# DefTruth/CUDA-Learn-Notes

Hardware: AMD Instinct MI355X
Metric: HGEMM fp16 TFLOPS at M=N=K=4096 (higher is better)
Workload: dtype f16; 1 GPU; HGEMM fp16 NN M=N=K=4096, stages=2, block swizzle stride 2048 (BASELINE config C3); kernel=hgemm_mma_m16n8k16_mma2x4_warp4x4x2_stages_dsmem, parallelism=replicas x1, launch=eager

## Files before the change

### cuda-learn-notes_amd/csrc/hgemm_w4.cuh

```cuda
#pragma once
#include <type_traits>

#include "hgemm_mfma.cuh"

namespace hgemm {

template <int FM, int FN, int NT = 0>
__device__ __forceinline__ void store_wide_tile_via_lds(half_t* Cmat, int N, int row0, int col0, int lane, char* wave_lds,
                                                        const f4 (&acc)[FM][FN], int nt_ok = 1) {
  static_assert(FN == 8 || FN == 6 || FN == 5 || FN == 4, "128-, 96-, 80- or 64-column wave tile");
  constexpr int RS = FN * 32 + 16;
  constexpr int LPR = FN * 2;
  constexpr int RPI = 64 / LPR;
#pragma unroll
  for (int h0 = 0; h0 < FM; h0 += 4) {
    constexpr int NF_FULL = 4;
    const int nf = FM - h0 < NF_FULL ? FM - h0 : NF_FULL;
#pragma unroll
    for (int i = 0; i < NF_FULL; ++i)
#pragma unroll
      for (int j = 0; j < FN; ++j) {
        if (i < nf) {
          const f4 v = acc[(h0 + i) < FM ? (h0 + i) : 0][j];
          h4 o = {(half_t)v[0], (half_t)v[1], (half_t)v[2], (half_t)v[3]};
          *reinterpret_cast<h4*>(wave_lds + (i * 16 + (lane & 15)) * RS + (j * 16 + 4 * (lane >> 4)) * 2) = o;
        }
      }
    const int rows = nf * 16;
#pragma unroll
    for (int it = 0; it < (64 + RPI - 1) / RPI; ++it) {
      const int r = it * RPI + lane / LPR;
      if (it * RPI < rows && lane < RPI * LPR && r < rows) {
        const u4 v = *reinterpret_cast<const u4*>(wave_lds + r * RS + (lane % LPR) * 16);
        u4* dst = reinterpret_cast<u4*>(Cmat + (size_t)(row0 + h0 * 16 + r) * N + col0 + (lane % LPR) * 8);
        if constexpr (NT == 1) {
          if (nt_ok) asm volatile("global_store_dwordx4 %0, %1, off nt\n\ts_nop 1" ::"v"(dst), "v"(v) : "memory");
          else asm volatile("global_store_dwordx4 %0, %1, off\n\ts_nop 1" ::"v"(dst), "v"(v) : "memory");
        } else if constexpr (NT == 3) asm volatile("global_store_dwordx4 %0, %1, off nt\n\ts_nop 1" ::"v"(dst), "v"(v) : "memory");
        else if constexpr (NT == 2) asm volatile("global_store_dwordx4 %0, %1, off sc0 sc1\n\ts_nop 1" ::"v"(dst), "v"(v) : "memory");
        else *dst = v;
      }
    }
  }
}

template <int FM, int FN>
__device__ __forceinline__ void store_wide_tile_via_lds_rows16(half_t* Cmat, int N, int row0, int col0, int lane, char* wave_lds, const f4 (&acc)[FM][FN],
                                                               int nt_ok) {
  static_assert(FN == 8, "128-column wave tile");
  constexpr int RS = FN * 32 + 16, LPR = FN * 2, RPI = 64 / LPR;
#pragma unroll
  for (int i = 0; i < FM; ++i) {
#pragma unroll
    for (int j = 0; j < FN; ++j) {
      const f4 v = acc[i][j];
      h4 o = {(half_t)v[0], (half_t)v[1], (half_t)v[2], (half_t)v[3]};
      *reinterpret_cast<h4*>(wave_lds + (lane & 15) * RS + (j * 16 + 4 * (lane >> 4)) * 2) = o;
    }
#pragma unroll
    for (int it = 0; it < 16 / RPI; ++it) {
      const int r = it * RPI + lane / LPR;
      const u4 v = *reinterpret_cast<const u4*>(wave_lds + r * RS + (lane % LPR) * 16);
      u4* dst = reinterpret_cast<u4*>(Cmat + (size_t)(row0 + i * 16 + r) * N + col0 + (lane % LPR) * 8);
      if (nt_ok) asm volatile("global_store_dwordx4 %0, %1, off nt\n\ts_nop 1" ::"v"(dst), "v"(v) : "memory");
      else asm volatile("global_store_dwordx4 %0, %1, off\n\ts_nop 1" ::"v"(dst), "v"(v) : "memory");
    }
    asm volatile("s_waitcnt lgkmcnt(0)" ::: "memory");
  }
}

template <int... Ns, typename F>
__device__ __forceinline__ void static_for_impl(std::integer_sequence<int, Ns...>, F&& f) {
  (f(std::integral_constant<int, Ns>{}), ...);
}
template <int N, typename F>
__device__ __forceinline__ void static_for(F&& f) {
  static_for_impl(std::make_integer_sequence<int, N>{}, f);
}

struct W4Sched {
  int r1_first, r1_step;
  int b1;
  int d_first, d_step;
  int b2;
  int r0_first, r0_step;
};
constexpr W4Sched w4_sched(int var) {
  switch (var) {
    case 1: return {1, 2, 36, 38, 4, 94, 96, 2};
    case 2: return {1, 2, 40, 42, 3, 94, 96, 2};
    case 3: return {1, 1, 24, 26, 4, 94, 96, 2};
    case 4: return {1, 2, 36, 38, 4, 102, 103, 1};
    case 5: return {1, 2, 36, 38, 5, 102, 103, 1};
    case 6: return {1, 1, 20, 22, 6, 102, 103, 1};
    case 7: return {1, 2, 36, 38, 4, 94, 95, 1};
    case 8: return {1, 1, 20, 22, 4, 94, 95, 1};
    case 9: return {1, 1, 20, 22, 5, 102, 103, 1};
    case 10: return {1, 2, 36, 38, 8, 102, 103, 1};
    case 11: return {1, 2, 36, 38, 7, 102, 103, 1};
    case 12: return {1, 2, 36, 40, 6, 102, 103, 1};
    case 13: return {1, 1, 36, 38, 4, 102, 103, 1};
    case 14: return {1, 1, 20, 38, 4, 102, 103, 1};
    default: return {1, 2, 40, 42, 2, 94, 96, 2};
  }
}
constexpr W4Sched w4_sched_for(int FM, int FN, int d_step) {
  const int NR = FM + FN, NM = 2 * FM * FN, b1 = 1 + 2 * (NR - 1) + 5, b2 = NM - NR - 10;
  return {1, 2, b1, b1 + 2, d_step, b2, b2 + 1, 1};
}

template <typename C, int NLOADS>
struct NFillW {
  unsigned voff[NLOADS];
  __device__ __forceinline__ void init(int N, int wave, int lane) {
    constexpr int LPR = C::BN / 8;
#pragma unroll
    for (int i = 0; i < NLOADS; ++i) {
      const int L = (i * C::NW + wave) * 64 + lane;
      const int krow = L / LPR, c = L % LPR;
      voff[i] = ((unsigned)krow * (unsigned)N + ((c ^ nswz_bn<C::BN>(krow)) << 3)) * 2u;
    }
  }
};
template <int BN>
__device__ __forceinline__ h8 read_nfrag_w(const char* img, int n0w, int lane, int kk) {
  const int i = lane & 15, g = lane >> 4;
  const int q = (n0w >> 3) + ((i & 3) >> 1);
  const int k_lo = kk * 32 + 8 * g + (i >> 2);
  const int k_hi = k_lo + 4;
  const char* p_lo = img + k_lo * (BN * 2) + ((q ^ nswz_bn<BN>(k_lo)) << 4) + ((i & 1) << 3);
  const char* p_hi = img + k_hi * (BN * 2) + ((q ^ nswz_bn<BN>(k_hi)) << 4) + ((i & 1) << 3);
  return h8_cat(lds_read_tr16(p_lo), lds_read_tr16(p_hi));
}

template <int BM_, int BN_, int LAYOUT_>
struct W4Cfg {
  static constexpr int BM = BM_, BN = BN_, BK = 64, NW = 4, LAYOUT = LAYOUT_;
  static constexpr int WTM = BM / 2, WTN = BN / 2, FM = WTM / 16, FN = WTN / 16;
  static constexpr int A_BYTES = BM * 128, B_BYTES = BN * 128, STAGE_BYTES = A_BYTES + B_BYTES, LDS_BYTES = 2 * STAGE_BYTES;
  static constexpr int A_LOADS = FM, B_LOADS = FN, NP = FM + FN;
  static constexpr int NR = FM + FN, NM = 2 * FM * FN;
  static_assert(((BM == 256 || BM == 192 || BM == 128) && (BN == 256 || BN == 192 || BN == 128) && BM + BN >= 384) ||
                    (BM == 160 && BN == 160),
                "wave tiles of 128, 96, 80 or 64 rows / columns; enough MFMAs per K tile to hang the schedule on");
};

constexpr int W4_TICKET_FLOATS = 1024;
template <int LAYOUT, int EPI = 2, int VAR = 0, int ABL = 0, int BM = 256, int BN = 256, bool ODD = false>
__global__ __launch_bounds__(256, 1) void hgemm_w4_kernel(const half_t* __restrict__ A, const half_t* __restrict__ B,
                                                          half_t* __restrict__ Cmat, int M, int N, int K, int tiles_m,
                                                          int tiles_n, int swizzle, int band, float* __restrict__ ws = nullptr) {
  using C = W4Cfg<BM, BN, LAYOUT>;
  constexpr bool SPLITK = EPI == 5 || EPI == 6;
  constexpr int FM = C::FM, FN = C::FN, NR = C::NR, NP = C::NP, NM = C::NM;
  constexpr W4Sched S = (BM == 256 && BN == 256) ? w4_sched(VAR & 15) : w4_sched_for(FM, FN, (BM == 128 || BN == 128 || BM == 160) ? 2 : (BM == 192 && BN == 192) ? 4 : 5);
  constexpr bool SNAKE = (VAR >> 4) & 1;
  static_assert(S.r0_first + (NR - 1) * S.r0_step < NM && S.r1_first + (NR - 1) * S.r1_step < S.b1 && S.b1 < S.d_first &&
                    S.b2 < S.r0_first && S.r0_first >= NM / 2 && (NP - 1) * S.d_step < NM && S.d_first + (NP - 1) * S.d_step - NM < S.d_first &&
                    S.d_first < NM && S.b2 >= S.d_first,
                "schedule: reads drained before B1, DMA after B1 and landed before the next B2, late pieces before early ones");
  constexpr int D_EARLY = (NM - 1 - S.d_first) / S.d_step + 1 > NP ? NP : (NM - 1 - S.d_first) / S.d_step + 1;
  constexpr int D_BEFORE_B2 = (S.b2 - S.d_first) / S.d_step + 1 > D_EARLY ? D_EARLY : (S.b2 - S.d_first) / S.d_step + 1;
  extern __shared__ __attribute__((aligned(16))) char smem[];
  const int lane = threadIdx.x & 63;
  const int wave = __builtin_amdgcn_readfirstlane(threadIdx.x >> 6);
  const int wm = wave >> 1, wn = wave & 1;
  constexpr bool PERSIST = EPI == 7;
  const int n_tiles = tiles_m * tiles_n;
  int tm, tn;
  auto coords = [&](int vb, int& tm_, int& tn_) {
    if (swizzle & 4) {
      tile_coords_interleaved(vb, PERSIST ? n_tiles : (int)gridDim.x, tiles_m, tiles_n, band, tm_, tn_);
    } else {
      tile_coords(vb, PERSIST ? n_tiles : (int)gridDim.x, tiles_m, tiles_n, swizzle & 1, band, tm_, tn_);
    }
  };
  int vb = blockIdx.x;
  coords(vb, tm, tn);
  int m0 = tm * BM, n0 = tn * BN;

  KFill<C, FM> fa;
  KFill<C, FN> fbt;
  NFillW<C, FN> fbn;
  const char* a_src;
  const char* b_src;
  if constexpr (SPLITK) {
    const int ld = (swizzle >> 8) * 64;
    const size_t k0 = (size_t)blockIdx.y * K;
    fa.init(ld, wave, lane);
    if constexpr (LAYOUT == TN) fbt.init(ld, wave, lane);
    else fbn.init(N, wave, lane);
    a_src = reinterpret_cast<const char*>(A + (size_t)m0 * ld + k0);
    b_src = (LAYOUT == TN) ? reinterpret_cast<const char*>(B + (size_t)n0 * ld + k0) : reinterpret_cast<const char*>(B + k0 * N + n0);
  } else {
    fa.init(K, wave, lane);
    if constexpr (LAYOUT == TN) fbt.init(K, wave, lane);
    else fbn.init(N, wave, lane);
    a_src = reinterpret_cast<const char*>(A + (size_t)m0 * K);
    b_src = (LAYOUT == TN) ? reinterpret_cast<const char*>(B + (size_t)n0 * K) : reinterpret_cast<const char*>(B + n0);
  }
  const size_t a_step = 128;
  const size_t b_step = (LAYOUT == TN) ? (size_t)128 : (size_t)64 * N * 2;
  const unsigned lds0 = lds_addr_of(smem);
  auto voff_of = [&](int p) -> unsigned {
    return p < FM ? fa.voff[p < FM ? p : 0] : (LAYOUT == TN ? fbt.voff[(p - FM) < FN ? (p - FM) : 0] : fbn.voff[(p - FM) < FN ? (p - FM) : 0]);
  };
  auto piece = [&](int p, unsigned img) { glds16_asm(p < FM ? a_src : b_src, voff_of(p), img + (unsigned)(p * 4 + wave) * 1024u); };
  const char* a_old = a_src;
  const char* b_old = b_src;
  auto piece_m0 = [&](int p, unsigned img, bool late, bool set_m0) {
    const unsigned voff = (ABL & 8) ? (unsigned)(lane * 16) : voff_of(p);
    const char* src = (ABL & 8) ? reinterpret_cast<const char*>(A) : late ? (p < FM ? a_old : b_old) : (p < FM ? a_src : b_src);
    if (set_m0)
      asm volatile("s_mov_b32 m0, %2\n\ts_nop 0\n\tglobal_load_lds_dwordx4 %0, %1\n\ts_add_u32 m0, m0, 0x1000"
                   :: "v"(voff), "s"(src), "s"(img + (unsigned)(p * 4 + wave) * 1024u) : "memory", "scc", "m0");
    else
      asm volatile("global_load_lds_dwordx4 %0, %1\n\ts_add_u32 m0, m0, 0x1000" :: "v"(voff), "s"(src) : "memory", "scc", "m0");
  };
  auto advance = [&]() {
    a_old = a_src;
    b_old = b_src;
    a_src += a_step;
    b_src += b_step;
  };

  f4 acc[FM][FN];
  h8 af[2][FM], bf[2][FN];
  bool prefetched = false;
  for (;;) {
#pragma unroll
  for (int i = 0; i < FM; ++i)
#pragma unroll
    for (int j = 0; j < FN; ++j) acc[i][j] = f4{0.f, 0.f, 0.f, 0.f};
#pragma unroll
  for (int i = 0; i < FM; ++i)
#pragma unroll
    for (int j = 0; j < FN; ++j) asm volatile("" : "+a"(acc[i][j]));
  asm volatile("s_nop 7");

  auto read_op = [&](const char* img, int kk, int r) {
    const char* bimg = img + C::A_BYTES;
    if (r == 0 || r > FN) {
      const int i = r == 0 ? 0 : r - FN;
      af[kk][i] = read_kfrag<64>(img, wm * C::WTM + i * 16 + (lane & 15), lane, kk);
    } else {
      const int j = r - 1;
      if constexpr (LAYOUT == TN) bf[kk][j] = read_kfrag<64>(bimg, wn * C::WTN + j * 16 + (lane & 15), lane, kk);
      else bf[kk][j] = read_nfrag_w<BN>(bimg, wn * C::WTN + j * 16, lane, kk);
    }
  };
#define W4_PIN() __builtin_amdgcn_sched_barrier(0)
#define W4_BARRIER()                 \
  do {                               \
    __builtin_amdgcn_s_barrier();    \
    asm volatile("" ::: "memory");   \
  } while (0)

  auto tile = [&](auto dma_c, auto late_c, auto next_c, const char* img, const char* nimg, unsigned img_lds, unsigned nimg_lds) {
    constexpr bool DMA = decltype(dma_c)::value, LATE = decltype(late_c)::value, NEXT = decltype(next_c)::value;
    static_for<NM>([&](auto nc) {
      constexpr int n = decltype(nc)::value;
      constexpr int kk = n / (FM * FN), idx = n % (FM * FN), i = idx / FN, lo0 = idx % FN;
      constexpr int j = (SNAKE && (i & 1)) ? FN - 1 - lo0 : lo0;
      asm volatile("v_mfma_f32_16x16x32_f16 %0, %1, %2, %0" : "+a"(acc[i][j]) : "v"(bf[kk][j]), "v"(af[kk][i]));
      constexpr bool R1 = n >= S.r1_first && (n - S.r1_first) % S.r1_step == 0 && (n - S.r1_first) / S.r1_step < NR;
      constexpr bool DP = DMA && n >= S.d_first && (n - S.d_first) % S.d_step == 0 && (n - S.d_first) / S.d_step < NP;
      constexpr int gl = n + NM;
      constexpr bool LP = LATE && (gl - S.d_first) % S.d_step == 0 && (gl - S.d_first) / S.d_step < NP && (gl - S.d_first) / S.d_step >= D_EARLY;
      constexpr bool R0 = NEXT && n >= S.r0_first && (n - S.r0_first) % S.r0_step == 0 && (n - S.r0_first) / S.r0_step < NR;
      if constexpr (R1 && !(ABL & 1)) read_op(img, 1, (n - S.r1_first) / S.r1_step);
      if constexpr (n == S.b1) {
        asm volatile("s_waitcnt lgkmcnt(0)" ::: "memory");
        if constexpr (!(ABL & 4)) W4_BARRIER();
      }
      if constexpr (LP && !(ABL & 2)) piece_m0((gl - S.d_first) / S.d_step, nimg_lds, true, (gl - S.d_first) / S.d_step == D_EARLY);
      if constexpr (DP && !(ABL & 2)) piece_m0((n - S.d_first) / S.d_step, img_lds, false, n == S.d_first);
      if constexpr (NEXT && n == S.b2) {
        if constexpr (DMA && !(ABL & 2)) wait_vmcnt<D_BEFORE_B2>();
        else wait_vmcnt<0>();
        if constexpr (!(ABL & 4)) W4_BARRIER();
      }
      if constexpr (R0 && !(ABL & 1)) read_op(nimg, 0, (n - S.r0_first) / S.r0_step);
      if constexpr (R1 || DP || LP || R0 || n == S.b1 || (NEXT && n == S.b2)) W4_PIN();
    });
    if constexpr (DMA) advance();
  };

  const int nt = K / 64;
  auto prologue_requests = [&]() {
#pragma unroll
    for (int p = 0; p < NP; ++p) piece(p, lds0);
    advance();
#pragma unroll
    for (int p = 0; p < NP; ++p) piece(p, lds0 + C::STAGE_BYTES);
    advance();
  };
  constexpr int C_STORES = FM * FN / 2;
  if (PERSIST && prefetched) {
    static_assert(C_STORES < 64, "vmcnt is a 6-bit field");
    wait_vmcnt<C_STORES>();
  } else {
    prologue_requests();
    wait_vmcnt<NP>();
  }
  W4_BARRIER();
#pragma unroll
  for (int r = 0; r < NR; ++r) read_op(smem, 0, r);
  W4_PIN();

  const char* img0 = smem;
  const char* img1 = smem + C::STAGE_BYTES;
  const unsigned lds1 = lds0 + C::STAGE_BYTES;
  constexpr std::true_type Y{};
  constexpr std::false_type NO{};
  tile(Y, NO, Y, img0, img1, lds0, lds1);
  tile(Y, Y, Y, img1, img0, lds1, lds0);
  int t = 2;
  do {
    tile(Y, Y, Y, img0, img1, lds0, lds1);
    tile(Y, Y, Y, img1, img0, lds1, lds0);
    t += 2;
  } while (t + (ODD ? 3 : 2) < nt);
  if constexpr (ODD) {
    tile(Y, Y, Y, img0, img1, lds0, lds1);
    tile(NO, Y, Y, img1, img0, lds1, lds0);
    tile(NO, NO, NO, img0, img1, lds0, lds1);
  } else {
    tile(NO, Y, Y, img0, img1, lds0, lds1);
    tile(NO, NO, NO, img1, img0, lds1, lds0);
  }
#undef W4_PIN
#undef W4_BARRIER
  asm volatile("s_nop 15\n\ts_nop 7" ::: "memory");
#pragma unroll
  for (int i = 0; i < FM; ++i)
#pragma unroll
    for (int j = 0; j < FN; ++j) asm volatile("" : "+a"(acc[i][j]));
  if constexpr (SPLITK) {
    const int tile = tm * tiles_n + tn, tiles = tiles_m * tiles_n;
    float* part = (EPI == 6 ? ws + W4_TICKET_FLOATS : reinterpret_cast<float*>(Cmat));
    float* dst = part + ((size_t)blockIdx.y * tiles + tile) * (BM * BN) + wave * (C::WTM * C::WTN) + lane * 4;
    if constexpr (EPI == 5) {
#pragma unroll
      for (int i = 0; i < FM; ++i)
#pragma unroll
        for (int j = 0; j < FN; ++j) *reinterpret_cast<f4*>(dst + (i * FN + j) * 256) = acc[i][j];
    }
    if constexpr (EPI == 6) {
#pragma unroll
      for (int i = 0; i < FM; ++i)
#pragma unroll
        for (int j = 0; j < FN; ++j) asm volatile("global_store_dwordx4 %0, %1, off sc1\n\ts_nop 1" ::"v"(dst + (i * FN + j) * 256), "v"(acc[i][j]) : "memory");
      asm volatile("s_waitcnt vmcnt(0)" ::: "memory");
      const int S = gridDim.y;
      int* last = reinterpret_cast<int*>(smem + C::LDS_BYTES - 16);
      __syncthreads();
      if (threadIdx.x == 0) {
        unsigned* tk = reinterpret_cast<unsigned*>(ws) + tile;
        const unsigned old = __hip_atomic_fetch_add(tk, 1u, __ATOMIC_RELAXED, __HIP_MEMORY_SCOPE_AGENT);
        const int l = old == (unsigned)(S - 1);
        if (l) __hip_atomic_store(tk, 0u, __ATOMIC_RELAXED, __HIP_MEMORY_SCOPE_AGENT);
        *last = l;
      }
      __syncthreads();
      if (*last == 0) return;
      const float* src = part + (size_t)tile * (BM * BN) + wave * (C::WTM * C::WTN) + lane * 4;
      const size_t split_stride = (size_t)tiles * (BM * BN);
#pragma unroll
      for (int i0 = 0; i0 < FM; i0 += 2) {
        for (int ks = 0; ks < S; ++ks) {
          const float* p = src + (size_t)ks * split_stride;
          f4 t[2][FN];
#pragma unroll
          for (int i = i0; i < i0 + 2 && i < FM; ++i)
#pragma unroll
            for (int j = 0; j < FN; ++j) asm volatile("global_load_dwordx4 %0, %1, off sc1" : "=v"(t[i - i0][j]) : "v"(p + (i * FN + j) * 256) : "memory");
          asm volatile("s_waitcnt vmcnt(0)" ::: "memory");
#pragma unroll
          for (int i = i0; i < i0 + 2 && i < FM; ++i)
#pragma unroll
            for (int j = 0; j < FN; ++j) {
              asm volatile("" : "+v"(t[i - i0][j]));
              acc[i][j] = ks == 0 ? t[i - i0][j] : acc[i][j] + t[i - i0][j];
            }
        }
      }
      store_wide_tile_via_lds<FM, FN, 0>(Cmat, N, m0 + wm * C::WTM, n0 + wn * C::WTN, lane, smem + wave * (64 * (FN * 32 + 16)), acc, 0);
    }
  } else if constexpr (PERSIST) {
    const int nvb = vb + (int)gridDim.x;
    const bool more = nvb < n_tiles;
    const int row0 = m0 + wm * C::WTM, col0 = n0 + wn * C::WTN;
    if (more) {
      coords(nvb, tm, tn);
      m0 = tm * BM, n0 = tn * BN;
      a_src = reinterpret_cast<const char*>(A + (size_t)m0 * K);
      b_src = (LAYOUT == TN) ? reinterpret_cast<const char*>(B + (size_t)n0 * K) : reinterpret_cast<const char*>(B + n0);
      prologue_requests();
    }
    store_wide_tile_via_lds_rows16<FM, FN>(Cmat, N, row0, col0, cln_fresh_lane(), smem + C::LDS_BYTES + wave * (16 * (FN * 32 + 16)), acc, (swizzle >> 1) & 1);
    if (!more) break;
    vb = nvb, prefetched = true;
    continue;
  } else if constexpr (EPI >= 2) {
    store_wide_tile_via_lds<FM, FN, EPI - 2>(Cmat, N, m0 + wm * C::WTM, n0 + wn * C::WTN, lane, smem + wave * (64 * (FN * 32 + 16)), acc, (swizzle >> 1) & 1);
  } else {
    float s = 0.f;
#pragma unroll
    for (int i = 0; i < FM; ++i)
#pragma unroll
      for (int j = 0; j < FN; ++j) s += acc[i][j][0] + acc[i][j][1] + acc[i][j][2] + acc[i][j][3];
    if (s == 123.456f) Cmat[(size_t)m0 * N + n0] = (half_t)s;
  }
  break;
  }
}

inline bool w4_k_ok(int K) { return K % 64 == 0 && K >= ((K / 64) & 1 ? 448 : 384); }
constexpr long long W4_NT_FOOTPRINT = 96LL << 20;
inline int w4_nt_ok(int M, int N, int K) { return 2LL * ((long long)M * K + (long long)K * N + (long long)M * N) >= W4_NT_FOOTPRINT ? 1 : 0; }
constexpr long long W4_INTERLEAVED_OPERANDS = 512LL << 20;
inline int w4_interleaved_walk(int M, int N, int K, int swizzle, int tiles) {
  if (!swizzle || tiles < 512) return 0;
  return (tiles >= 1024 && 2LL * ((long long)M * K + (long long)K * N) >= W4_INTERLEAVED_OPERANDS) ? 1 : 0;
}
inline int w4_swizzle_arg(int M, int N, int K, int swizzle, int tiles) { return (swizzle ? 1 : 0) | (w4_nt_ok(M, N, K) << 1) | (w4_interleaved_walk(M, N, K, swizzle, tiles) << 2); }
inline int w4_grid(int, int, int, int, int tiles_m, int tiles_n) { return tiles_m * tiles_n; }

template <int LAYOUT, int EPI = 2, int VAR = 0, int ABL = 0, int BM = 256, int BN = 256>
int launch_w4(const void* a, const void* b, void* c, int M, int N, int K, int swizzle, int swizzle_stride,
              hipStream_t stream) {
  using C = W4Cfg<BM, BN, LAYOUT>;
  constexpr bool HAS_ODD = ABL == 0 && EPI >= 2 && (VAR == 26 || BM != 256 || BN != 256);
  const bool odd = (K / 64) & 1;
  if (M % BM || N % BN || !w4_k_ok(K) || (odd && !HAS_ODD)) return CLN_ERR_UNSUPPORTED;
  const int tiles_m = M / BM, tiles_n = N / BN;
  int band = (swizzle && swizzle_stride >= BN) ? swizzle_stride / BN : tiles_n;
  if constexpr (HAS_ODD) {
    if (odd) {
      static cln_lds_attr lds_attr_odd;
      if (cln_ensure_lds(lds_attr_odd, reinterpret_cast<const void*>(&hgemm_w4_kernel<LAYOUT, EPI, VAR, ABL, BM, BN, true>), C::LDS_BYTES) != CLN_OK)
        return CLN_ERR_LAUNCH;
      CLN_LAUNCH((hgemm_w4_kernel<LAYOUT, EPI, VAR, ABL, BM, BN, true>), dim3(w4_grid(M, N, K, swizzle, tiles_m, tiles_n)), dim3(256), C::LDS_BYTES, stream,
                 (const half_t*)a, (const half_t*)b, (half_t*)c, M, N, K, tiles_m, tiles_n, w4_swizzle_arg(M, N, K, swizzle, tiles_m * tiles_n), band);
      return cln_check_launch();
    }
  }
  static cln_lds_attr lds_attr;
  if (cln_ensure_lds(lds_attr, reinterpret_cast<const void*>(&hgemm_w4_kernel<LAYOUT, EPI, VAR, ABL, BM, BN>), C::LDS_BYTES) != CLN_OK)
    return CLN_ERR_LAUNCH;
  CLN_LAUNCH((hgemm_w4_kernel<LAYOUT, EPI, VAR, ABL, BM, BN>), dim3(w4_grid(M, N, K, swizzle, tiles_m, tiles_n)), dim3(256), C::LDS_BYTES, stream,
             (const half_t*)a, (const half_t*)b, (half_t*)c, M, N, K, tiles_m, tiles_n, w4_swizzle_arg(M, N, K, swizzle, tiles_m * tiles_n), band);
  return cln_check_launch();
}

inline int w4_cu_count() {
  static const int n = [] {
    int dev = 0, cus = 256;
    if (hipGetDevice(&dev) == hipSuccess) (void)hipDeviceGetAttribute(&cus, hipDeviceAttributeMultiprocessorCount, dev);
    (void)hipGetLastError();
    return cus > 0 ? cus & ~7 : 256;
  }();
  return n;
}
template <int LAYOUT, int VAR = 26>
int launch_w4_persist(const void* a, const void* b, void* c, int M, int N, int K, int swizzle, int swizzle_stride, hipStream_t stream) {
  constexpr int BM = 256, BN = 256, EPI = 7;
  using C = W4Cfg<BM, BN, LAYOUT>;
  constexpr int LDS = C::LDS_BYTES + 4 * 16 * (C::FN * 32 + 16);
  static_assert(LDS <= 160 * 1024, "ring + epilogue staging rows");
  const bool odd = (K / 64) & 1;
  if (M % BM || N % BN || !w4_k_ok(K)) return CLN_ERR_UNSUPPORTED;
  const int tiles_m = M / BM, tiles_n = N / BN, tiles = tiles_m * tiles_n;
  const int band = (swizzle && swizzle_stride >= BN) ? swizzle_stride / BN : tiles_n;
  const int grid = tiles < w4_cu_count() ? tiles : w4_cu_count();
  if (odd) {
    static cln_lds_attr lds_attr_odd;
    if (cln_ensure_lds(lds_attr_odd, reinterpret_cast<const void*>(&hgemm_w4_kernel<LAYOUT, EPI, VAR, 0, BM, BN, true>), LDS) != CLN_OK) return CLN_ERR_LAUNCH;
    CLN_LAUNCH((hgemm_w4_kernel<LAYOUT, EPI, VAR, 0, BM, BN, true>), dim3(grid), dim3(256), LDS, stream, (const half_t*)a, (const half_t*)b, (half_t*)c, M, N, K,
               tiles_m, tiles_n, w4_swizzle_arg(M, N, K, swizzle, tiles), band);
  } else {
    static cln_lds_attr lds_attr;
    if (cln_ensure_lds(lds_attr, reinterpret_cast<const void*>(&hgemm_w4_kernel<LAYOUT, EPI, VAR, 0, BM, BN>), LDS) != CLN_OK) return CLN_ERR_LAUNCH;
    CLN_LAUNCH((hgemm_w4_kernel<LAYOUT, EPI, VAR, 0, BM, BN>), dim3(grid), dim3(256), LDS, stream, (const half_t*)a, (const half_t*)b, (half_t*)c, M, N, K,
               tiles_m, tiles_n, w4_swizzle_arg(M, N, K, swizzle, tiles), band);
  }
  return cln_check_launch();
}

}
```

### cuda-learn-notes_amd/csrc/probe/hgemm_probe.hip

```cpp
#include "hgemm_dispatch.h"
#include "hgemm_mfma.cuh"
#include "hgemm_w4.cuh"
#include "hgemm_w4s.cuh"
#include "hgemm_splitk.cuh"

using namespace hgemm;

namespace {
int check_args(const void* a, const void* b, const void* c, int M, int N, int K) {
  if (!a || !b || !c) return CLN_ERR_BAD_ARG;
  if (M <= 0 || N <= 0 || K <= 0) return CLN_ERR_BAD_ARG;
  if (!cln_aligned16(a) || !cln_aligned16(b) || !cln_aligned16(c)) return CLN_ERR_BAD_ARG;
  return CLN_OK;
}
using C1S_128_NN = Cfg<128, 128, 32, 2, 2, 1, NN>;
}

CLN_API int cln_hgemm_variant(int kind, int layout, int tile, int bk, int stages, const void* a, const void* b,
                              void* c, int M, int N, int K, int swizzle, int swizzle_stride, void* stream_) {
  int rc = check_args(a, b, c, M, N, K);
  if (rc != CLN_OK) return rc;
  hipStream_t stream = (hipStream_t)stream_;
  if (kind == 0) {
    return layout == TN ? ring_exact_tn(tile, bk, stages, a, b, c, M, N, K, swizzle, swizzle_stride, stream)
                        : ring_exact_nn(tile, bk, stages, a, b, c, M, N, K, swizzle, swizzle_stride, stream);
  }
  if (kind == 1) {
    return layout == TN ? launch_1stage<Cfg<128, 128, 32, 2, 2, 1, TN>>(a, b, c, M, N, K, stream)
                        : launch_1stage<C1S_128_NN>(a, b, c, M, N, K, stream);
  }
  if (kind == 3) {
    return layout == TN ? launch_pp<TN>(a, b, c, M, N, K, swizzle, swizzle_stride, stream)
                        : launch_pp<NN>(a, b, c, M, N, K, swizzle, swizzle_stride, stream);
  }
  if (kind == 4) return launch_pp<NN, 1>(a, b, c, M, N, K, swizzle, swizzle_stride, stream);
  if (kind == 5) {
    if (stages == 4)
      return layout == TN ? launch_pp<TN, 2, 4>(a, b, c, M, N, K, swizzle, swizzle_stride, stream)
                          : launch_pp<NN, 2, 4>(a, b, c, M, N, K, swizzle, swizzle_stride, stream);
    return layout == TN ? launch_pp<TN, 2, 8>(a, b, c, M, N, K, swizzle, swizzle_stride, stream)
                        : launch_pp<NN, 2, 8>(a, b, c, M, N, K, swizzle, swizzle_stride, stream);
  }
  if (kind == 8) {
    if (stages == 1) return launch_pp<NN, 1, 4, 0, 1>(a, b, c, M, N, K, swizzle, swizzle_stride, stream);
    return layout == TN ? launch_pp<TN, 2, 4, 0, 1>(a, b, c, M, N, K, swizzle, swizzle_stride, stream)
                        : launch_pp<NN, 2, 4, 0, 1>(a, b, c, M, N, K, swizzle, swizzle_stride, stream);
  }
  if (kind == 9) {
    if (stages == 1) return launch_pp32<NN, 1>(a, b, c, M, N, K, swizzle, swizzle_stride, stream);
    return layout == TN ? launch_pp32<TN, 2>(a, b, c, M, N, K, swizzle, swizzle_stride, stream)
                        : launch_pp32<NN, 2>(a, b, c, M, N, K, swizzle, swizzle_stride, stream);
  }
  if (kind == 10) {
    if (stages == 1) return launch_m32<NN, 1>(a, b, c, M, N, K, swizzle, swizzle_stride, stream);
    if (stages >= 16) {
      switch (stages - 16) {
        case 1: return launch_m32<NN, 1, 1>(a, b, c, M, N, K, swizzle, swizzle_stride, stream);
        case 2: return launch_m32<NN, 1, 2>(a, b, c, M, N, K, swizzle, swizzle_stride, stream);
        case 3: return launch_m32<NN, 1, 3>(a, b, c, M, N, K, swizzle, swizzle_stride, stream);
        case 7: return launch_m32<NN, 1, 7>(a, b, c, M, N, K, swizzle, swizzle_stride, stream);
        case 8: return launch_m32<NN, 2, 8>(a, b, c, M, N, K, swizzle, swizzle_stride, stream);
        default: return CLN_ERR_BAD_ARG;
      }
    }
    return layout == TN ? launch_m32<TN>(a, b, c, M, N, K, swizzle, swizzle_stride, stream)
                        : launch_m32<NN>(a, b, c, M, N, K, swizzle, swizzle_stride, stream);
  }
  if (kind == 11) {
    if (stages == 1) return layout == TN ? launch_pp<TN, 2, 4, 0, 0, 256>(a, b, c, M, N, K, swizzle, swizzle_stride, stream)
                                         : launch_pp<NN, 2, 4, 0, 0, 256>(a, b, c, M, N, K, swizzle, swizzle_stride, stream);
    return layout == TN ? launch_pp<TN, 2, 4, 0, 0, 192>(a, b, c, M, N, K, swizzle, swizzle_stride, stream)
                        : launch_pp<NN, 2, 4, 0, 0, 192>(a, b, c, M, N, K, swizzle, swizzle_stride, stream);
  }
  if (kind == 12) {
    if (stages == 2) return layout == TN ? launch_pp<TN, 2, 2, 0, 0, 192>(a, b, c, M, N, K, swizzle, swizzle_stride, stream)
                                         : launch_pp<NN, 2, 2, 0, 0, 192>(a, b, c, M, N, K, swizzle, swizzle_stride, stream);
    return layout == TN ? launch_pp<TN, 2, 2, 0, 0, 256>(a, b, c, M, N, K, swizzle, swizzle_stride, stream)
                        : launch_pp<NN, 2, 2, 0, 0, 256>(a, b, c, M, N, K, swizzle, swizzle_stride, stream);
  }
  if (kind == 13) {
    if (stages == 2) return layout == TN ? launch_pp<TN, 2, 4, 0, 2, 192>(a, b, c, M, N, K, swizzle, swizzle_stride, stream)
                                         : launch_pp<NN, 2, 4, 0, 2, 192>(a, b, c, M, N, K, swizzle, swizzle_stride, stream);
    return layout == TN ? launch_pp<TN, 2, 4, 0, 2, 256>(a, b, c, M, N, K, swizzle, swizzle_stride, stream)
                        : launch_pp<NN, 2, 4, 0, 2, 256>(a, b, c, M, N, K, swizzle, swizzle_stride, stream);
  }
  if (kind == 14) {
#define W4_CASE(V)                                                                                         \
  case V: return layout == TN ? launch_w4<TN, 2, V>(a, b, c, M, N, K, swizzle, swizzle_stride, stream)    \
                              : launch_w4<NN, 2, V>(a, b, c, M, N, K, swizzle, swizzle_stride, stream);
    switch (stages) {
      W4_CASE(0) W4_CASE(1) W4_CASE(3) W4_CASE(4) W4_CASE(9) W4_CASE(10) W4_CASE(13)
      W4_CASE(20) W4_CASE(25) W4_CASE(26) W4_CASE(27) W4_CASE(28)
      case 104: return layout == TN ? launch_w4<TN, 1, 4>(a, b, c, M, N, K, swizzle, swizzle_stride, stream)
                                    : launch_w4<NN, 1, 4>(a, b, c, M, N, K, swizzle, swizzle_stride, stream);
      case 203: return layout == TN ? launch_w4<TN, 3, 26>(a, b, c, M, N, K, swizzle, swizzle_stride, stream)
                                    : launch_w4<NN, 3, 26>(a, b, c, M, N, K, swizzle, swizzle_stride, stream);
      case 204: return layout == TN ? launch_w4<TN, 4, 26>(a, b, c, M, N, K, swizzle, swizzle_stride, stream)
                                    : launch_w4<NN, 4, 26>(a, b, c, M, N, K, swizzle, swizzle_stride, stream);
      case 111: return launch_w4<NN, 1, 4, 1>(a, b, c, M, N, K, swizzle, swizzle_stride, stream);
      case 112: return launch_w4<NN, 1, 4, 2>(a, b, c, M, N, K, swizzle, swizzle_stride, stream);
      case 113: return launch_w4<NN, 1, 4, 3>(a, b, c, M, N, K, swizzle, swizzle_stride, stream);
      case 114: return launch_w4<NN, 1, 4, 4>(a, b, c, M, N, K, swizzle, swizzle_stride, stream);
      case 118: return launch_w4<NN, 1, 4, 8>(a, b, c, M, N, K, swizzle, swizzle_stride, stream);
      case 117: return launch_w4<NN, 1, 4, 7>(a, b, c, M, N, K, swizzle, swizzle_stride, stream);
      default: return CLN_ERR_BAD_ARG;
    }
#undef W4_CASE
  }
  if (kind == 15) {
#define W4_SHAPE(BM, BN)                                                                                              \
  return layout == TN ? launch_w4<TN, 2, 26, 0, BM, BN>(a, b, c, M, N, K, swizzle, swizzle_stride, stream)           \
                      : launch_w4<NN, 2, 26, 0, BM, BN>(a, b, c, M, N, K, swizzle, swizzle_stride, stream);
    if (tile == 0) { W4_SHAPE(192, 256) }
    if (tile == 1) { W4_SHAPE(256, 192) }
    if (tile == 2) { W4_SHAPE(192, 192) }
    if (tile == 3) { W4_SHAPE(128, 256) }
    if (tile == 4) { W4_SHAPE(256, 128) }
    if (tile == 5) { W4_SHAPE(160, 160) }
#undef W4_SHAPE
    return CLN_ERR_BAD_ARG;
  }
  if (kind == 16) {
#define W4S_CASE(SS)                                                                                     \
  case SS: return layout == TN ? launch_w4s<TN, SS>(a, b, c, M, N, K, swizzle, swizzle_stride, stream)   \
                               : launch_w4s<NN, SS>(a, b, c, M, N, K, swizzle, swizzle_stride, stream);
    switch (stages) {
      W4S_CASE(2) W4S_CASE(3) W4S_CASE(4) W4S_CASE(5)
      default: return CLN_ERR_BAD_ARG;
    }
#undef W4S_CASE
  }
  if (kind == 17) {
    static float* ws = nullptr;
    constexpr size_t WS_BYTES = 512u << 20;
    if (!ws && hipMalloc(&ws, WS_BYTES) != hipSuccess) return ws = nullptr, CLN_ERR_LAUNCH;
    if ((size_t)stages * M * N * 4 > WS_BYTES) return CLN_ERR_UNSUPPORTED;
#define SK_SHAPE(TT, BMM, BNN)                                                                                              \
  if (tile == TT) return layout == TN ? launch_w4_splitk<TN, 26, BMM, BNN>(a, b, c, ws, M, N, K, stages, stream)           \
                                      : launch_w4_splitk<NN, 26, BMM, BNN>(a, b, c, ws, M, N, K, stages, stream);
    SK_SHAPE(0, 256, 256) SK_SHAPE(1, 128, 256) SK_SHAPE(2, 256, 128) SK_SHAPE(3, 192, 256) SK_SHAPE(4, 192, 192) SK_SHAPE(5, 160, 160)
#undef SK_SHAPE
    return CLN_ERR_BAD_ARG;
  }
  if (kind == 20) {
    static float* ws = nullptr;
    constexpr size_t WS_BYTES = 512u << 20;
    if (!ws) {
      if (hipMalloc(&ws, WS_BYTES + W4_TICKET_FLOATS * 4) != hipSuccess) return ws = nullptr, CLN_ERR_LAUNCH;
      if (hipMemset(ws, 0, W4_TICKET_FLOATS * 4) != hipSuccess) return CLN_ERR_LAUNCH;
    }
    if ((size_t)stages * M * N * 4 > WS_BYTES) return CLN_ERR_UNSUPPORTED;
#define SKF_SHAPE(TT, BMM, BNN)                                                                                                  \
  if (tile == TT) return layout == TN ? launch_w4_splitk_fused<TN, 26, BMM, BNN>(a, b, c, ws, M, N, K, stages, stream)           \
                                      : launch_w4_splitk_fused<NN, 26, BMM, BNN>(a, b, c, ws, M, N, K, stages, stream);
    SKF_SHAPE(0, 256, 256) SKF_SHAPE(1, 128, 256) SKF_SHAPE(3, 192, 256) SKF_SHAPE(4, 192, 192) SKF_SHAPE(5, 160, 160)
#undef SKF_SHAPE
    return CLN_ERR_BAD_ARG;
  }
  if (kind == 18) {
    static float* ws = nullptr;
    constexpr size_t WS_BYTES = 512u << 20;
    if (!ws && hipMalloc(&ws, WS_BYTES) != hipSuccess) return ws = nullptr, CLN_ERR_LAUNCH;
    if ((size_t)stages * tile * 256 * N * 4 > WS_BYTES) return CLN_ERR_UNSUPPORTED;
    const int m_split = M - tile * 256;
    return layout == TN ? launch_w4_tail_split<TN, 3, 26, 256, 256>(a, b, c, ws, M, N, K, m_split, stages, swizzle, swizzle_stride, stream)
                        : launch_w4_tail_split<NN, 3, 26, 256, 256>(a, b, c, ws, M, N, K, m_split, stages, swizzle, swizzle_stride, stream);
  }
  if (kind == 19) return layout == TN ? launch_w4_persist<TN>(a, b, c, M, N, K, swizzle, swizzle_stride, stream) : launch_w4_persist<NN>(a, b, c, M, N, K, swizzle, swizzle_stride, stream);
  if (kind == 6) return launch_pp<NN, 1, 4>(a, b, c, M, N, K, swizzle, swizzle_stride, stream);
  if (kind == 7) {
    switch (stages) {
      case 1: return launch_pp<NN, 1, 4, 1>(a, b, c, M, N, K, swizzle, swizzle_stride, stream);
      case 2: return launch_pp<NN, 1, 4, 2>(a, b, c, M, N, K, swizzle, swizzle_stride, stream);
      case 3: return launch_pp<NN, 1, 4, 3>(a, b, c, M, N, K, swizzle, swizzle_stride, stream);
      case 7: return launch_pp<NN, 1, 4, 7>(a, b, c, M, N, K, swizzle, swizzle_stride, stream);
      case 8: return launch_pp<NN, 1, 4, 8>(a, b, c, M, N, K, swizzle, swizzle_stride, stream);
      case 4: return launch_pp<NN, 1, 4, 4>(a, b, c, M, N, K, swizzle, swizzle_stride, stream);
      default: return CLN_ERR_BAD_ARG;
    }
  }
  if (kind == 2) return layout == TN ? launch_naive<TN>(a, b, c, M, N, K, stream) : launch_naive<NN>(a, b, c, M, N, K, stream);
  return CLN_ERR_BAD_ARG;
}
```

Before: 1402 TFLOPS.

## Issue prologue loads before accumulator init and double-buffer the epilogue stores

Moves the prologue global-to-LDS load requests ahead of accumulator zeroing, with a scheduling barrier, so memory latency overlaps setup work. It also adds a two-buffer, row-16 epilogue for 128-column wave tiles that converts the next fragment row into LDS while the current row's global stores are in flight. Ablation bits and probe cases are added to switch each part off. The double-buffered epilogue uses a different LDS staging layout per wave and relies on the order of LDS writes and reads without an explicit lgkmcnt wait, which carries correctness and hazard risk.

```diff
diff --git a/cuda-learn-notes_amd/csrc/hgemm_w4.cuh b/cuda-learn-notes_amd/csrc/hgemm_w4.cuh
--- a/cuda-learn-notes_amd/csrc/hgemm_w4.cuh
+++ b/cuda-learn-notes_amd/csrc/hgemm_w4.cuh
@@ -4,6 +4,15 @@
 #include "hgemm_mfma.cuh"
 
 namespace hgemm {
+
+template <int... Ns, typename F>
+__device__ __forceinline__ void static_for_impl(std::integer_sequence<int, Ns...>, F&& f) {
+  (f(std::integral_constant<int, Ns>{}), ...);
+}
+template <int N, typename F>
+__device__ __forceinline__ void static_for(F&& f) {
+  static_for_impl(std::make_integer_sequence<int, N>{}, f);
+}
 
 template <int FM, int FN, int NT = 0>
 __device__ __forceinline__ void store_wide_tile_via_lds(half_t* Cmat, int N, int row0, int col0, int lane, char* wave_lds,
@@ -44,11 +53,45 @@
   }
 }
 
-template <int FM, int FN>
+template <int FM, int FN, int NT = 1, int NBUF = 1>
 __device__ __forceinline__ void store_wide_tile_via_lds_rows16(half_t* Cmat, int N, int row0, int col0, int lane, char* wave_lds, const f4 (&acc)[FM][FN],
                                                                int nt_ok) {
   static_assert(FN == 8, "128-column wave tile");
+  static_assert(NBUF == 1 || NBUF == 2, "one staging region or two");
   constexpr int RS = FN * 32 + 16, LPR = FN * 2, RPI = 64 / LPR;
+  if constexpr (NBUF == 2) {
+    constexpr int SPR = 16 / RPI, FPS = FN / SPR;
+    static_assert(SPR * FPS == FN, "whole fragments per store");
+    auto put = [&](auto ic, int j) {
+      constexpr int i = decltype(ic)::value;
+      const f4 v = acc[i][j];
+      h4 o = {(half_t)v[0], (half_t)v[1], (half_t)v[2], (half_t)v[3]};
+      *reinterpret_cast<h4*>(wave_lds + (i & 1) * (16 * RS) + (lane & 15) * RS + (j * 16 + 4 * (lane >> 4)) * 2) = o;
+    };
+#pragma unroll
+    for (int j = 0; j < FN; ++j) put(std::integral_constant<int, 0>{}, j);
+    static_for<FM>([&](auto ic) {
+      constexpr int i = decltype(ic)::value;
+      u4 v[SPR];
+#pragma unroll
+      for (int it = 0; it < SPR; ++it) v[it] = *reinterpret_cast<const u4*>(wave_lds + (i & 1) * (16 * RS) + (it * RPI + lane / LPR) * RS + (lane % LPR) * 16);
+#pragma unroll
+      for (int it = 0; it < SPR; ++it) {
+        u4* dst = reinterpret_cast<u4*>(Cmat + (size_t)(row0 + i * 16 + it * RPI + lane / LPR) * N + col0 + (lane % LPR) * 8);
+        if constexpr (NT == 1) {
+          if (nt_ok) asm volatile("global_store_dwordx4 %0, %1, off nt\n\ts_nop 1" ::"v"(dst), "v"(v[it]) : "memory");
+          else asm volatile("global_store_dwordx4 %0, %1, off\n\ts_nop 1" ::"v"(dst), "v"(v[it]) : "memory");
+        } else if constexpr (NT == 3) asm volatile("global_store_dwordx4 %0, %1, off nt\n\ts_nop 1" ::"v"(dst), "v"(v[it]) : "memory");
+        else if constexpr (NT == 2) asm volatile("global_store_dwordx4 %0, %1, off sc0 sc1\n\ts_nop 1" ::"v"(dst), "v"(v[it]) : "memory");
+        else *dst = v[it];
+        if constexpr (i + 1 < FM) {
+#pragma unroll
+          for (int j = it * FPS; j < it * FPS + FPS; ++j) put(std::integral_constant<int, (i + 1 < FM ? i + 1 : 0)>{}, j);
+        }
+      }
+    });
+    return;
+  }
 #pragma unroll
   for (int i = 0; i < FM; ++i) {
 #pragma unroll
@@ -67,15 +110,6 @@
     }
     asm volatile("s_waitcnt lgkmcnt(0)" ::: "memory");
   }
-}
-
-template <int... Ns, typename F>
-__device__ __forceinline__ void static_for_impl(std::integer_sequence<int, Ns...>, F&& f) {
-  (f(std::integral_constant<int, Ns>{}), ...);
-}
-template <int N, typename F>
-__device__ __forceinline__ void static_for(F&& f) {
-  static_for_impl(std::make_integer_sequence<int, N>{}, f);
 }
 
 struct W4Sched {
@@ -224,10 +258,30 @@
     b_src += b_step;
   };
 
+  auto prologue_requests = [&]() {
+#pragma unroll
+    for (int p = 0; p < NP; ++p) {
+      if constexpr (PERSIST || (ABL & 32)) piece(p, lds0);
+      else piece_m0(p, lds0, false, p == 0);
+    }
+    advance();
+#pragma unroll
+    for (int p = 0; p < NP; ++p) {
+      if constexpr (PERSIST || (ABL & 32)) piece(p, lds0 + C::STAGE_BYTES);
+      else piece_m0(p, lds0 + C::STAGE_BYTES, false, p == 0);
+    }
+    advance();
+  };
+  constexpr bool REQUEST_FIRST = !PERSIST && !(ABL & 16);
+
   f4 acc[FM][FN];
   h8 af[2][FM], bf[2][FN];
   bool prefetched = false;
   for (;;) {
+  if constexpr (REQUEST_FIRST) {
+    prologue_requests();
+    __builtin_amdgcn_sched_barrier(0);
+  }
 #pragma unroll
   for (int i = 0; i < FM; ++i)
 #pragma unroll
@@ -287,20 +341,12 @@
   };
 
   const int nt = K / 64;
-  auto prologue_requests = [&]() {
-#pragma unroll
-    for (int p = 0; p < NP; ++p) piece(p, lds0);
-    advance();
-#pragma unroll
-    for (int p = 0; p < NP; ++p) piece(p, lds0 + C::STAGE_BYTES);
-    advance();
-  };
   constexpr int C_STORES = FM * FN / 2;
   if (PERSIST && prefetched) {
     static_assert(C_STORES < 64, "vmcnt is a 6-bit field");
     wait_vmcnt<C_STORES>();
   } else {
-    prologue_requests();
+    if constexpr (!REQUEST_FIRST) prologue_requests();
     wait_vmcnt<NP>();
   }
   W4_BARRIER();
@@ -403,7 +449,10 @@
     vb = nvb, prefetched = true;
     continue;
   } else if constexpr (EPI >= 2) {
-    store_wide_tile_via_lds<FM, FN, EPI - 2>(Cmat, N, m0 + wm * C::WTM, n0 + wn * C::WTN, lane, smem + wave * (64 * (FN * 32 + 16)), acc, (swizzle >> 1) & 1);
+    if constexpr (FN == 8 && !(ABL & 64))
+      store_wide_tile_via_lds_rows16<FM, FN, EPI - 2, 2>(Cmat, N, m0 + wm * C::WTM, n0 + wn * C::WTN, lane, smem + wave * (2 * 16 * (FN * 32 + 16)), acc, (swizzle >> 1) & 1);
+    else
+      store_wide_tile_via_lds<FM, FN, EPI - 2>(Cmat, N, m0 + wm * C::WTM, n0 + wn * C::WTN, lane, smem + wave * (64 * (FN * 32 + 16)), acc, (swizzle >> 1) & 1);
   } else {
     float s = 0.f;
 #pragma unroll
diff --git a/cuda-learn-notes_amd/csrc/probe/hgemm_probe.hip b/cuda-learn-notes_amd/csrc/probe/hgemm_probe.hip
--- a/cuda-learn-notes_amd/csrc/probe/hgemm_probe.hip
+++ b/cuda-learn-notes_amd/csrc/probe/hgemm_probe.hip
@@ -103,6 +103,10 @@
       case 114: return launch_w4<NN, 1, 4, 4>(a, b, c, M, N, K, swizzle, swizzle_stride, stream);
       case 118: return launch_w4<NN, 1, 4, 8>(a, b, c, M, N, K, swizzle, swizzle_stride, stream);
       case 117: return launch_w4<NN, 1, 4, 7>(a, b, c, M, N, K, swizzle, swizzle_stride, stream);
+      case 316: return launch_w4<NN, 3, 26, 16>(a, b, c, M, N, K, swizzle, swizzle_stride, stream);
+      case 332: return launch_w4<NN, 3, 26, 32>(a, b, c, M, N, K, swizzle, swizzle_stride, stream);
+      case 364: return launch_w4<NN, 3, 26, 64>(a, b, c, M, N, K, swizzle, swizzle_stride, stream);
+      case 412: return launch_w4<NN, 3, 26, 112>(a, b, c, M, N, K, swizzle, swizzle_stride, stream);
       default: return CLN_ERR_BAD_ARG;
     }
 #undef W4_CASE
```

After: 1415 TFLOPS, median of 6. About the same (+0.9%).
